# damaggu/StableKeypoints

Measured on AMD Instinct MI355X. Metric: images/sec (token-opt step, 512², N=500 tokens), higher is better.
Workload: dtype f32

## Files before the change

### include/skp.h

```cpp
#ifndef SKP_H
#define SKP_H

#ifdef __cplusplus
extern "C" {
#endif

#define SKP_OK 0
#define SKP_EBADARG (-1)
#define SKP_ELAUNCH (-2)
#define SKP_MAX_LAYERS 16

const char* skp_last_error(void);
int skp_version(void);

int skp_capture_fwd(const float* z_low, int BH, int s, int N, int R, float* attn, float* stats, void* stream);

int skp_capture_bwd(const float* z_low, int BH, int s, int N, int R, const float* dattn, int group, long long sb,
                    long long sp, long long sn, float gscale, const float* stats, float* dz_low, float* workspace,
                    void* stream);

int skp_capture_maps_fwd(const float* const* z_low, const int* sizes, int L, int B, int H, int N, int R, float* maps,
                         float* const* stats, void* stream);

int skp_capture_maps_bwd(const float* const* z_low, const int* sizes, int L, int B, int H, int N, int R,
                         const float* dmaps, float gscale, const float* const* stats, float* const* dz_low,
                         float* workspace, void* stream);

long long skp_capture_maps_bwd_sel_workspace(const int* sizes, int L, int B, int H, int N, int R, int K);
int skp_capture_maps_bwd_sel(const float* const* z_low, const int* sizes, int L, int B, int H, int N, int R,
                             const long long* sel_tok, int K, const float* gsel, float gscale,
                             const float* const* stats, float* const* dz_low, float* workspace, void* stream);
int skp_sel_bwd_timing(int enable);
int skp_sel_bwd_timing_read(double* ms, int* calls);

int skp_aggregate(const float* const* layers, int L, int BH, int RR, int N, const long long* indices,
                  int n_out, float* out, void* stream);

int skp_resize_bilinear(const float* in, int C, int R, int Ro, float* out, void* stream);
int skp_resize_bilinear_bwd(const float* gout, int C, int R, int Ro, float* gin, void* stream);

int skp_argmax2d(const float* maps, int T, int h, int w, const long long* rows, int n_rows, float* pos,
                 long long* idx, void* stream);

int skp_k_max_pixels(const float* maps, int T, int h, int w, int num, float radius2, float* pos,
                     float* masked, void* stream);

int skp_mask_radius(const float* maps, int T, int h, int w, const float* pos, float radius2, float* out,
                    void* stream);

int skp_weighted_avg(float* maps, int T, int h, int w, float distance, int mutate, float* pos, void* stream);

int skp_gaussian_target(const float* pos, int num, int T, int size, float sigma, float* out, void* stream);

int skp_topk_gaussian(const float* maps, int T, int h, int w, int top_k, float sigma, float epsilon,
                      int num_subjects, long long* out, double* kl, void* workspace, void* stream);

int skp_topk_gaussian_batch(const float* maps, int nb, int T, int h, int w, int top_k, float sigma,
                            float epsilon, int num_subjects, long long* out, double* kl, void* workspace,
                            void* stream);

int skp_topk_keys(const double* keys, int nb, int T, int top_k, long long* out, void* stream);

int skp_entropy_sort(const float* maps, int T, int h, int w, int top_k, long long* out, double* ent,
                     void* workspace, void* stream);

int skp_fps(const float* maps, int T, int h, int w, const long long* cand, int n_cand, int top_k,
            long long* out, int* n_out, void* workspace, void* stream);
int skp_fps_batch(const float* maps, int nb, int T, int h, int w, const long long* cand, int n_cand, int top_k,
                  long long* out, int* n_out, void* workspace, void* stream);
int skp_fps_keys_batch(const double* keys, const float* maps, int nb, int T, int h, int w, int n_cand, int top_k,
                       long long* cand, long long* out, int* n_out, void* workspace, void* stream);

int skp_sharpen_fwd(const float* A, int T, int h, int w, float sigma, int num_subjects, float* pos,
                     double* partial, float* loss, void* stream);
int skp_sharpen_bwd(const float* A, int T, int h, int w, float sigma, int num_subjects, const float* pos,
                     const float* gout, float* dA, void* stream);
int skp_sharpen_fwd_batch(const float* A, int nb, int T, int h, int w, float sigma, int num_subjects, float* pos,
                          double* partial, float* loss, void* stream);
int skp_sharpen_bwd_batch(const float* A, int nb, int T, int h, int w, float sigma, int num_subjects,
                          const float* pos, const float* gout, float* dA, void* stream);

int skp_affine_warp(const float* x, int B, int C, int H, int W, const float* theta, float* out, void* stream);
int skp_affine_warp_bwd(const float* gout, int B, int C, int H, int W, const float* theta, float* gin,
                        void* stream);

int skp_equiv_fwd(const float* A, const float* At, int T, int h, int w, const float* theta_inv,
                  double* partial, float* loss, void* stream);
int skp_equiv_bwd(const float* A, const float* At, int T, int h, int w, const float* theta_inv,
                  const float* gout, float* dA, float* dAt, void* stream);
int skp_equiv_fwd_batch(const float* A, const float* At, int nb, int T, int h, int w, const float* theta_inv,
                        double* partial, float* loss, void* stream);
int skp_equiv_bwd_batch(const float* A, const float* At, int nb, int T, int h, int w, const float* theta_inv,
                        const float* gout, float* dA, float* dAt, void* stream);

int skp_wino_in_transform(const float* x, int B, int C, int H, int W, float* V, void* stream);
int skp_wino_out_transform(const float* M, int B, int K, int H, int W, const float* bias, const float* residual,
                           float* y, void* stream);
int skp_wino_out_transform_kt(const float* M, int B, int K, int H, int W, const float* bias, const float* residual,
                              float* y, float* gn_part, void* stream);

int skp_bgemm_f32(const float* A, long long sAb, long long sAm, long long sAk, const float* B, long long sBb,
                  long long sBk, long long sBn, float* C, long long sCb, long long sCm, long long sCn, int batch,
                  int M, int N, int K, float alpha, int accumulate, void* stream);
int skp_bgemm_f32_2b(const float* A, long long sAo, long long sAb, long long sAm, long long sAk, const float* B,
                     long long sBo, long long sBb, long long sBk, long long sBn, float* C, long long sCo, long long sCb,
                     long long sCm, long long sCn, int batch, int hb, int M, int N, int K, float alpha, int accumulate,
                     void* stream);

int skp_groupnorm_workspace(int B, int C, long long HW, int G);
int skp_groupnorm_fwd(const float* x, const float* gamma, const float* beta, const float* shift, int B, int C,
                      long long HW, int G, float eps, int act, float* y, float* stats, double* partial,
                      void* stream);
int skp_groupnorm_bwd(const float* x, const float* dy, const float* gamma, const float* beta, const float* shift,
                      const float* stats, int B, int C, long long HW, int G, int act, float* dx, double* partial,
                      void* stream);
int skp_groupnorm_fwd_part(const float* x, const float* gamma, const float* beta, const float* shift, const float* part,
                           int nseg, int B, int C, long long HW, int G, float eps, int act, float* y, float* stats,
                           double* partial, void* stream);
int skp_groupnorm_stats(const float* x, const float* shift, int B, int C, long long HW, int G, float eps, float* stats,
                        double* partial, void* stream);
int skp_groupnorm_stats_part(const float* part, int nseg, const float* shift, int B, int C, long long HW, int G,
                             float eps, float* stats, double* partial, void* stream);
int skp_groupnorm_bwd_add(const float* x, const float* dy, const float* gamma, const float* beta, const float* shift,
                          const float* stats, int B, int C, long long HW, int G, int act, const float* dres, float* dx,
                          double* partial, void* stream);
int skp_softmax_bwd(const float* P, float* dP, long long rows, int cols, float alpha, void* stream);
int skp_softmax_fwd(float* S, long long rows, int cols, void* stream);
int skp_attn_dscore(const float* P, const float* dO, const float* V, const float* D, float* out, int BH, int S, int L,
                    int d, float alpha, void* stream);
int skp_attn_bwd_kv(const float* P, const float* dO, const float* Q, const float* V, const float* D, float* dS,
                    float* dV, float* dK, int BH, int S, int L, int d, float alpha, void* stream);
int skp_attn_fwd(const float* Q, const float* K, const float* V, float* O, float* stats, int BH, int S, int L, int d,
                 float scale, void* stream);
int skp_attn_bwd_flash(const float* Q, const float* K, const float* V, const float* dO, const float* stats,
                       const float* D, float* dS, float* dV, float* dK, int BH, int S, int L, int d, float scale,
                       void* stream);
int skp_attn_fwd_bshd(const float* Q, long long q_sb, int q_rs, const float* K, long long k_sb, int k_rs,
                      const float* V, long long v_sb, int v_rs, float* O, long long o_sb, int o_rs, float* stats, int B,
                      int H, int S, int L, int d, float scale, void* stream);
int skp_attn_bwd_flash_bshd(const float* Q, long long q_sb, int q_rs, const float* K, long long k_sb, int k_rs,
                            const float* V, long long v_sb, int v_rs, const float* dO, long long o_sb, int o_rs,
                            const float* stats, const float* D, float* dS, float* dV, long long dv_sb, int dv_rs,
                            float* dK, long long dk_sb, int dk_rs, int B, int H, int S, int L, int d, float scale,
                            void* stream);
int skp_layernorm_fwd(const float* x, const float* gamma, const float* beta, long long rows, int C, float eps, float* y,
                      float* stats, void* stream);
int skp_layernorm_bwd(const float* x, const float* dy, const float* gamma, const float* stats, long long rows, int C,
                      float* dx, void* stream);
int skp_layernorm_bwd_add(const float* x, const float* dy, const float* gamma, const float* stats, long long rows,
                          int C, const float* dres, float* dx, void* stream);
int skp_geglu_fwd(const float* h, long long rows, int I, float* out, void* stream);
int skp_geglu_bwd(const float* h, const float* dout, long long rows, int I, float* dh, void* stream);
int skp_residual_bias_add(const float* a, const float* h, const float* bias, int B, int C, long long HW,
                          float* out, void* stream);
int skp_wino_weights(const float* w, int K, int C, int flip, float* U, void* stream);
int skp_conv3x3_wino(const float* x, const float* U, const float* bias, const float* residual, float* y, int B, int C,
                     int K, int H, int W, int nsplit, float* ws, void* stream);
int skp_wino2_weights(const float* w, int K, int C, int flip, float* U, void* stream);
int skp_conv3x3_wino2(const float* x, const float* U, const float* bias, const float* residual, float* y, int B,
                      int C, int K, int H, int W, int nsplit, float* ws, void* stream);
int skp_conv3x3_wino2_gn(const float* x, const float* U, const float* bias, const float* residual, float* y, int B,
                         int C, int K, int H, int W, int nsplit, float* ws, float* gn_part, void* stream);
int skp_wino2_vtransform(const float* x, float* V, int B, int C, int H, int W, void* stream);
int skp_wino2_vtransform_gn(const float* x, const float* stats, const float* gamma, const float* beta,
                            const float* shift, int G, int act, float* V, int B, int C, int H, int W, void* stream);
int skp_conv3x3_wino2_v(const float* V, const float* U, const float* bias, const float* residual, float* y, int B,
                        int C, int K, int H, int W, int nsplit, float* ws, void* stream);
int skp_conv3x3_wino2_v_gn(const float* V, const float* U, const float* bias, const float* residual, float* y, int B,
                           int C, int K, int H, int W, int nsplit, float* ws, float* gn_part, void* stream);
int skp_wino2s2_weights(const float* w, int K, int C, float* U, void* stream);
int skp_conv3x3s2_f2(const float* x, const float* U, const float* bias, float* y, int B, int C, int K, int H, int W,
                     int nsplit, float* ws, void* stream);

int skp_map_range(const float* maps, int n, int h, int w, float* range, void* stream);
int skp_render_sheet(const float* images, int n, int H, int W, const float* maps, int h, int w, const float* range,
                     const float* lut, float alpha, const float* points, int K, float radius,
                     const unsigned char* colors, int rows, int cols, int f, int pad, unsigned char* out,
                     void* stream);

int skp_tta_reduce_workspace(int B, int n, int S);
int skp_tta_reduce(const float* maps, int B, int C, int n, int S, const float* theta_inv, float* pos, float* avg,
                   void* workspace, void* stream);

int skp_tta_reduce_scored_workspace(int B, int n, int S);
int skp_tta_reduce_scored(const float* maps, int B, int C, int n, int S, const float* theta_inv, float distance,
                          float* pos, float* refined, float* scores, float* avg, void* workspace, void* stream);

int skp_tta_reduce_peaks_workspace(int B, int n, int S, int num, float radius2);
int skp_tta_reduce_peaks(const float* maps, int B, int C, int n, int S, const float* theta_inv, int num,
                         float radius2, float* pos, float* values, float* avg, void* workspace, void* stream);
// ... 6 lines not shown
```

### stablekeypoints_amd/_lib.py

```python
import ctypes
import os

import torch

_HERE = os.path.dirname(os.path.abspath(__file__))
LIB_PATH = os.environ.get("SKP_LIB", os.path.join(_HERE, "libskp.so"))

_c_int, _c_float, _c_ll, _p = ctypes.c_int, ctypes.c_float, ctypes.c_longlong, ctypes.c_void_p

_SIGS = {
    "skp_capture_fwd": [_p, _c_int, _c_int, _c_int, _c_int, _p, _p, _p],
    "skp_capture_bwd": [_p, _c_int, _c_int, _c_int, _c_int, _p, _c_int, _c_ll, _c_ll, _c_ll, _c_float, _p, _p, _p,
                        _p],
    "skp_capture_maps_fwd": [ctypes.POINTER(_p), ctypes.POINTER(_c_int), _c_int, _c_int, _c_int, _c_int, _c_int, _p,
                             ctypes.POINTER(_p), _p],
    "skp_capture_maps_bwd": [ctypes.POINTER(_p), ctypes.POINTER(_c_int), _c_int, _c_int, _c_int, _c_int, _c_int, _p,
                             _c_float, ctypes.POINTER(_p), ctypes.POINTER(_p), _p, _p],
    "skp_capture_maps_bwd_sel": [ctypes.POINTER(_p), ctypes.POINTER(_c_int), _c_int, _c_int, _c_int, _c_int, _c_int,
                                 _p, _c_int, _p, _c_float, ctypes.POINTER(_p), ctypes.POINTER(_p), _p, _p],
    "skp_sel_bwd_timing": [_c_int],
    "skp_sel_bwd_timing_read": [_p, _p],
    "skp_capture_maps_bwd_sel_workspace": [ctypes.POINTER(_c_int), _c_int, _c_int, _c_int, _c_int, _c_int, _c_int],
    "skp_aggregate": [ctypes.POINTER(_p), _c_int, _c_int, _c_int, _c_int, _p, _c_int, _p, _p],
    "skp_resize_bilinear": [_p, _c_int, _c_int, _c_int, _p, _p],
    "skp_resize_bilinear_bwd": [_p, _c_int, _c_int, _c_int, _p, _p],
    "skp_argmax2d": [_p, _c_int, _c_int, _c_int, _p, _c_int, _p, _p, _p],
    "skp_k_max_pixels": [_p, _c_int, _c_int, _c_int, _c_int, _c_float, _p, _p, _p],
    "skp_mask_radius": [_p, _c_int, _c_int, _c_int, _p, _c_float, _p, _p],
    "skp_weighted_avg": [_p, _c_int, _c_int, _c_int, _c_float, _c_int, _p, _p],
    "skp_gaussian_target": [_p, _c_int, _c_int, _c_int, _c_float, _p, _p],
    "skp_topk_gaussian": [_p, _c_int, _c_int, _c_int, _c_int, _c_float, _c_float, _c_int, _p, _p, _p, _p],
    "skp_topk_gaussian_batch": [_p, _c_int, _c_int, _c_int, _c_int, _c_int, _c_float, _c_float, _c_int, _p, _p, _p,
                                _p],
    "skp_topk_keys": [_p, _c_int, _c_int, _c_int, _p, _p],
    "skp_entropy_sort": [_p, _c_int, _c_int, _c_int, _c_int, _p, _p, _p, _p],
    "skp_fps": [_p, _c_int, _c_int, _c_int, _p, _c_int, _c_int, _p, _p, _p, _p],
    "skp_fps_batch": [_p, _c_int, _c_int, _c_int, _c_int, _p, _c_int, _c_int, _p, _p, _p, _p],
    "skp_fps_keys_batch": [_p, _p, _c_int, _c_int, _c_int, _c_int, _c_int, _c_int, _p, _p, _p, _p, _p],
    "skp_sharpen_fwd": [_p, _c_int, _c_int, _c_int, _c_float, _c_int, _p, _p, _p, _p],
    "skp_sharpen_bwd": [_p, _c_int, _c_int, _c_int, _c_float, _c_int, _p, _p, _p, _p],
    "skp_wino_in_transform": [_p, _c_int, _c_int, _c_int, _c_int, _p, _p],
    "skp_wino_out_transform": [_p, _c_int, _c_int, _c_int, _c_int, _p, _p, _p, _p],
    "skp_wino_out_transform_kt": [_p, _c_int, _c_int, _c_int, _c_int, _p, _p, _p, _p, _p],
    "skp_sharpen_fwd_batch": [_p, _c_int, _c_int, _c_int, _c_int, _c_float, _c_int, _p, _p, _p, _p],
    "skp_sharpen_bwd_batch": [_p, _c_int, _c_int, _c_int, _c_int, _c_float, _c_int, _p, _p, _p, _p],
    "skp_affine_warp": [_p, _c_int, _c_int, _c_int, _c_int, _p, _p, _p],
    "skp_affine_warp_bwd": [_p, _c_int, _c_int, _c_int, _c_int, _p, _p, _p],
    "skp_equiv_fwd": [_p, _p, _c_int, _c_int, _c_int, _p, _p, _p, _p],
    "skp_equiv_bwd": [_p, _p, _c_int, _c_int, _c_int, _p, _p, _p, _p, _p],
    "skp_equiv_fwd_batch": [_p, _p, _c_int, _c_int, _c_int, _c_int, _p, _p, _p, _p],
    "skp_equiv_bwd_batch": [_p, _p, _c_int, _c_int, _c_int, _c_int, _p, _p, _p, _p, _p],
    "skp_bgemm_f32": [_p, _c_ll, _c_ll, _c_ll, _p, _c_ll, _c_ll, _c_ll, _p, _c_ll, _c_ll, _c_ll, _c_int, _c_int,
                      _c_int, _c_int, _c_float, _c_int, _p],
    "skp_bgemm_f32_2b": [_p, _c_ll, _c_ll, _c_ll, _c_ll, _p, _c_ll, _c_ll, _c_ll, _c_ll, _p, _c_ll, _c_ll, _c_ll,
                         _c_ll, _c_int, _c_int, _c_int, _c_int, _c_int, _c_float, _c_int, _p],
    "skp_groupnorm_workspace": [_c_int, _c_int, _c_ll, _c_int],
    "skp_groupnorm_fwd": [_p, _p, _p, _p, _c_int, _c_int, _c_ll, _c_int, _c_float, _c_int, _p, _p, _p, _p],
    "skp_groupnorm_bwd": [_p, _p, _p, _p, _p, _p, _c_int, _c_int, _c_ll, _c_int, _c_int, _p, _p, _p],
    "skp_groupnorm_bwd_add": [_p, _p, _p, _p, _p, _p, _c_int, _c_int, _c_ll, _c_int, _c_int, _p, _p, _p, _p],
    "skp_residual_bias_add": [_p, _p, _p, _c_int, _c_int, _c_ll, _p, _p],
    "skp_softmax_bwd": [_p, _p, _c_ll, _c_int, _c_float, _p],
    "skp_softmax_fwd": [_p, _c_ll, _c_int, _p],
    "skp_attn_dscore": [_p, _p, _p, _p, _p, _c_int, _c_int, _c_int, _c_int, _c_float, _p],
    "skp_attn_bwd_kv": [_p, _p, _p, _p, _p, _p, _p, _p, _c_int, _c_int, _c_int, _c_int, _c_float, _p],
    "skp_attn_fwd": [_p, _p, _p, _p, _p, _c_int, _c_int, _c_int, _c_int, _c_float, _p],
    "skp_attn_bwd_flash": [_p, _p, _p, _p, _p, _p, _p, _p, _p, _c_int, _c_int, _c_int, _c_int, _c_float, _p],
    "skp_attn_fwd_bshd": [_p, _c_ll, _c_int, _p, _c_ll, _c_int, _p, _c_ll, _c_int, _p, _c_ll, _c_int, _p, _c_int, _c_int,
                          _c_int, _c_int, _c_int, _c_float, _p],
    "skp_attn_bwd_flash_bshd": [_p, _c_ll, _c_int, _p, _c_ll, _c_int, _p, _c_ll, _c_int, _p, _c_ll, _c_int, _p, _p, _p,
                                _p, _c_ll, _c_int, _p, _c_ll, _c_int, _c_int, _c_int, _c_int, _c_int, _c_int, _c_float,
                                _p],
    "skp_layernorm_fwd": [_p, _p, _p, _c_ll, _c_int, _c_float, _p, _p, _p],
    "skp_layernorm_bwd": [_p, _p, _p, _p, _c_ll, _c_int, _p, _p],
    "skp_layernorm_bwd_add": [_p, _p, _p, _p, _c_ll, _c_int, _p, _p, _p],
    "skp_geglu_fwd": [_p, _c_ll, _c_int, _p, _p],
    "skp_geglu_bwd": [_p, _p, _c_ll, _c_int, _p, _p],
    "skp_wino_weights": [_p, _c_int, _c_int, _c_int, _p, _p],
    "skp_conv3x3_wino": [_p, _p, _p, _p, _p, _c_int, _c_int, _c_int, _c_int, _c_int, _c_int, _p, _p],
    "skp_wino2_weights": [_p, _c_int, _c_int, _c_int, _p, _p],
    "skp_conv3x3_wino2": [_p, _p, _p, _p, _p, _c_int, _c_int, _c_int, _c_int, _c_int, _c_int, _p, _p],
    "skp_conv3x3_wino2_gn": [_p, _p, _p, _p, _p, _c_int, _c_int, _c_int, _c_int, _c_int, _c_int, _p, _p, _p],
    "skp_groupnorm_fwd_part": [_p, _p, _p, _p, _p, _c_int, _c_int, _c_int, _c_ll, _c_int, _c_float, _c_int, _p, _p, _p,
                               _p],
    "skp_groupnorm_stats": [_p, _p, _c_int, _c_int, _c_ll, _c_int, _c_float, _p, _p, _p],
    "skp_groupnorm_stats_part": [_p, _c_int, _p, _c_int, _c_int, _c_ll, _c_int, _c_float, _p, _p, _p],
    "skp_wino2_vtransform": [_p, _p, _c_int, _c_int, _c_int, _c_int, _p],
    "skp_wino2_vtransform_gn": [_p, _p, _p, _p, _p, _c_int, _c_int, _p, _c_int, _c_int, _c_int, _c_int, _p],
    "skp_conv3x3_wino2_v": [_p, _p, _p, _p, _p, _c_int, _c_int, _c_int, _c_int, _c_int, _c_int, _p, _p],
    "skp_conv3x3_wino2_v_gn": [_p, _p, _p, _p, _p, _c_int, _c_int, _c_int, _c_int, _c_int, _c_int, _p, _p, _p],
    "skp_wino2s2_weights": [_p, _c_int, _c_int, _p, _p],
    "skp_conv3x3s2_f2":   [_p, _p, _p, _p, _c_int, _c_int, _c_int, _c_int, _c_int, _c_int, _p, _p],
    "skp_map_range": [_p, _c_int, _c_int, _c_int, _p, _p],
    "skp_render_sheet": [_p, _c_int, _c_int, _c_int, _p, _c_int, _c_int, _p, _p, _c_float, _p, _c_int, _c_float, _p,
                         _c_int, _c_int, _c_int, _c_int, _p, _p],
    "skp_tta_reduce_workspace": [_c_int, _c_int, _c_int],
    "skp_tta_reduce": [_p, _c_int, _c_int, _c_int, _c_int, _p, _p, _p, _p, _p],
    "skp_tta_reduce_scored_workspace": [_c_int, _c_int, _c_int],
    "skp_tta_reduce_scored": [_p, _c_int, _c_int, _c_int, _c_int, _p, _c_float, _p, _p, _p, _p, _p, _p],
    "skp_tta_reduce_peaks_workspace": [_c_int, _c_int, _c_int, _c_int, _c_float],
    "skp_tta_reduce_peaks": [_p, _c_int, _c_int, _c_int, _c_int, _p, _c_int, _c_float, _p, _p, _p, _p, _p],
    "skp_version": [],
}


_RESTYPE = {"skp_capture_maps_bwd_sel_workspace": _c_ll}
_MEASUREMENT_ONLY = {"skp_sel_bwd_timing", "skp_sel_bwd_timing_read"}


class SkpLibraryError(RuntimeError):
    pass


_lib = None


def lib():
    global _lib
    if _lib is None:
        if not os.path.exists(LIB_PATH):
            raise SkpLibraryError(f"libskp.so not found at {LIB_PATH}: build it with "
                                  "`python -c 'import __graft_entry__ as g; g.build()'` or `make -C stablekeypoints_amd/csrc`")
        try:
            L = ctypes.CDLL(LIB_PATH)
        except OSError as e:
            raise SkpLibraryError(f"cannot load {LIB_PATH}: {e}") from e
        for name, args in _SIGS.items():
            if name in _MEASUREMENT_ONLY and not hasattr(L, name):
                continue
            f = getattr(L, name)
            f.argtypes = args
            f.restype = _RESTYPE.get(name, _c_int)
        L.skp_last_error.argtypes = []
        L.skp_last_error.restype = ctypes.c_char_p
        _lib = L
    return _lib


def exported_symbols():
# ... 24 lines not shown
```

### stablekeypoints_amd/ops.py

```python
import ctypes
import os

import torch

from . import _lib
from ._lib import call, ptr, stream

F32 = torch.float32

_TIMER = None


def set_kernel_timer(timer):
    global _TIMER
    _TIMER = timer


class _NoTimer:
    def __enter__(self):
        return self

    def __exit__(self, *a):
        return False

# ... 1226 lines not shown

class QKVProjection(torch.autograd.Function):

    @staticmethod
    def forward(ctx, x, w3, C):
        out = torch.matmul(x, w3.t())
        ctx.save_for_backward(w3)
        ctx.C = C
        ctx.x_shape = x.shape
        ctx.set_materialize_grads(False)
        return tuple(out[..., i * C:(i + 1) * C] for i in range(w3.shape[0] // C))

    @staticmethod
    def backward(ctx, *grads):
        (w3,) = ctx.saved_tensors
        C = ctx.C
        dx = None
        for i, g in enumerate(grads):
            if g is None:
                continue
            g2 = g.reshape(-1, C)
            wi = w3[i * C:(i + 1) * C]
            if dx is None:
                dx = torch.mm(g2, wi)
            else:
                dx.addmm_(g2, wi)
        if dx is None:
            return None, None, None
        return dx.view(ctx.x_shape), None, None


QKV_FUSED = True


def qkv_projection(x, *ws):
    _lib.require_device(x)
    return QKVProjection.apply(x, _qkv_weight(*ws), int(ws[0].shape[0]))


class TokensProjIn(torch.autograd.Function):

    @staticmethod
    def forward(ctx, x, w, bias):
        B, C, HW = x.shape
        h = torch.bmm(x.transpose(1, 2), w.t().expand(B, C, w.shape[0]))
        if bias is not None:
            h.add_(bias)
        ctx.save_for_backward(w)
        return h

    @staticmethod
    def backward(ctx, dh):
        (w,) = ctx.saved_tensors
        B = dh.shape[0]
        dx = torch.bmm(w.t().expand(B, w.shape[1], w.shape[0]), dh.transpose(1, 2))
        return dx, None, None


class TokensProjOut(torch.autograd.Function):

    @staticmethod
    def forward(ctx, h, w):
        B = h.shape[0]
        ctx.save_for_backward(w)
        return torch.bmm(w.expand(B, *w.shape), h.transpose(1, 2))

    @staticmethod
    def backward(ctx, dy):
        (w,) = ctx.saved_tensors
        B = dy.shape[0]
        return torch.bmm(dy.transpose(1, 2), w.expand(B, *w.shape)), None


def tokens_proj_in(x, weight, bias):
    B, C = x.shape[:2]
    return TokensProjIn.apply(x.reshape(B, C, -1), weight.detach().reshape(weight.shape[0], C),
                              None if bias is None else bias.detach())


def tokens_proj_out(h, weight, bias, residual):
    B, C = residual.shape[:2]
    y = TokensProjOut.apply(h, weight.detach().reshape(C, h.shape[-1]))
    return residual_bias_add(residual, y.view(residual.shape), bias)


import weakref as _weakref

_WINO_U = {}
WINO_MIN_WORKGROUPS = 128
WINO_KERNEL = "auto"
WINO_SPLIT = True
WINO_NSPLIT_FORCE = 0


def _wino_v2(H, W, B=None):
    if WINO_KERNEL == "v1":
        return False
    return (H % 32 == 0 and W % 32 == 0) or (H == 16 and W == 16 and B is not None and B % 4 == 0)


def _wino_u_cached(weight, flip, form, build):
    key = id(weight)
    ent = _WINO_U.get(key)
    if ent is None or ent[0]() is not weight:
        ent = _WINO_U[key] = (_weakref.ref(weight, lambda _r: _WINO_U.pop(key, None)), {})
    hit = ent[1].get((flip, form))
    if hit is None or hit[0] != weight._version:
        hit = ent[1][(flip, form)] = (weight._version, build())
    return hit[1]


def _wino_u(weight, flip, v2=False):
    def build():
        w = _c(weight.detach())
        K, C = (w.shape[0], w.shape[1]) if not flip else (w.shape[1], w.shape[0])
        if v2 == "s2":
            U = torch.empty(K * C * 28, device=w.device, dtype=F32)
            call("skp_wino2s2_weights", ptr(w), K, C, ptr(U), stream(w.device))
        else:
            U = torch.empty(K * C * (40 if v2 else 36), device=w.device, dtype=F32)
            call("skp_wino2_weights" if v2 else "skp_wino_weights", ptr(w), K, C, int(flip), ptr(U), stream(w.device))
        return U
    return _wino_u_cached(weight, flip, v2, build)


def _batch_chunks(B, per_img_bytes):
    bmax = max(1, (2 ** 31 - 1) // per_img_bytes)
    for b0 in range(0, B, bmax):
        yield b0, min(B, b0 + bmax)


def _wino_plan_uncached(B, C, K, H, W, force):
    v2 = _wino_v2(H, W, B)
    if v2:
        wgs = (B // 4 if H == 16 else B * (H // 32) * (W // 32)) * (K // 32)
    elif B * (H // 4) * (W // 4) <= 32 and K % 64 == 0:
        wgs = K // 64
    else:
        wgs = -(-(B * (H // 4) * (W // 4)) // 64) * (K // 32)
    out_bytes = B * K * H * W * 4

    def cost(s):
        if v2:
            k = -(-2 * wgs * s // 256)
            st = C // s // 4
            return (k // 2) * st * 1.72e-6 + (k % 2) * st * 1.48e-6 + (s > 1) * (s + 1) * out_bytes / 2e12
        rounds = -(-wgs * s // 256)
        return rounds * ((C // s // 4) * 2.4e-6 + 5e-6) + (s > 1) * (s + 1) * out_bytes / 5e12

    nsplit = 1
    if WINO_SPLIT:
        cands = [s for s in range(1, 33) if C % (4 * s) == 0 and (s == 1 or C // s >= 32)]
        nsplit = min(cands, key=cost)
        if force and C % (4 * force) == 0:
            nsplit = force
    return v2, nsplit, wgs * nsplit


_WINO_PLANS = {}


def _wino_plan(B, C, K, H, W):
    force = int(WINO_NSPLIT_FORCE)
    key = (B, C, K, H, W, force, WINO_KERNEL, WINO_SPLIT)
    plan = _WINO_PLANS.get(key)
    if plan is None:
# ... 444 lines not shown
```

### stablekeypoints_amd/sd/unet.py

```python
import math

import os

import torch
import torch.nn as nn
import torch.nn.functional as F


class CaptureComplete(Exception):
    """Raised by a patched attention when its controller has every map it needs.

    The reference discards the UNet output of a capture pass
    (``ptp_utils.py:246-252``), and nothing after the 4th captured layer feeds the
    loss, so the forward may stop there (SURVEY.md §7 "UNet early exit").
    """


USE_FUSED_GROUPNORM = True
USE_SKP_LAYERNORM = True


def _fused(x, *modules):
    return USE_FUSED_GROUPNORM and x.is_cuda and not any(p.requires_grad for m in modules for p in m.parameters())

# ... 76 lines not shown
                qf = self.to_q(x)
                one = _shared_context(context)
                if one is not None:
                    k1, v1 = shared_kv(self, one)
                    kf, vf = k1.expand(x.shape[0], -1, -1), v1.expand(x.shape[0], -1, -1)
                else:
                    kf, vf = kv_projection(self, context)
            out = ops.attention_heads(qf, kf, vf, self.heads, self.scale)
            if out is None and one is not None and SHARED_HEAD_MAJOR and torch.is_grad_enabled():
                out = shared_context_attention(qf, k1, v1, self.heads, self.scale)
            if out is not None:
                return self.to_out[1](self.to_out[0](out))
            q = self.reshape_heads_to_batch_dim(qf)
            k, v = kf, vf
        else:
            q = self.reshape_heads_to_batch_dim(self.to_q(x))
            k, v = kv_projection(self, context)
        k = self.reshape_heads_to_batch_dim(k)
        v = self.reshape_heads_to_batch_dim(v)
        out = attention_core(q, k, v, self.scale, mask, self.heads)
        out = self.reshape_batch_dim_to_heads(out)
        return self.to_out[1](self.to_out[0](out))


SHARED_KV = True
SHARED_HEAD_MAJOR = True


def _shared_context(context):
    if SHARED_KV and context.dim() == 3 and context.shape[0] > 1 and context.stride(0) == 0:
        base = context._base
        if (base is not None and base.dim() == 3 and base.shape[0] == 1 and base.shape[1:] == context.shape[1:]
                and base.stride()[1:] == context.stride()[1:] and base.data_ptr() == context.data_ptr()):
            return base
        return context[:1]
    return None


def shared_kv(attn, one):
    from .. import ops
    if ops.QKV_FUSED and _fused(one, attn.to_k, attn.to_v) and attn.to_k.bias is None and attn.to_v.bias is None:
        return ops.qkv_projection(one, attn.to_k.weight, attn.to_v.weight)
    return attn.to_k(one), attn.to_v(one)


def shared_context_attention(qf, k1, v1, H, scale):
    B, S, C = qf.shape
    L, d = k1.shape[1], C // H
    q = qf.reshape(B, S, H, d).permute(2, 0, 1, 3).reshape(H, B * S, d)
    k = k1.reshape(L, H, d).transpose(0, 1).contiguous()
    v = v1.reshape(L, H, d).transpose(0, 1).contiguous()
    o = attention_core(q, k, v, scale)
    return o.reshape(H, B, S, d).permute(1, 2, 0, 3).reshape(B, S, C)


def kv_projection(attn, context):
    one = _shared_context(context)
    if one is not None:
        B = context.shape[0]
        k1, v1 = shared_kv(attn, one)
        return k1.expand(B, -1, -1), v1.expand(B, -1, -1)
    return attn.to_k(context), attn.to_v(context)


def attention_core(q, k, v, scale, mask=None, heads=1):
    if mask is None and CrossAttention.backend == "sdpa":
        return F.scaled_dot_product_attention(q.unsqueeze(0), k.unsqueeze(0), v.unsqueeze(0), scale=scale)[0]
    if mask is None and USE_FUSED_GROUPNORM and q.is_cuda and torch.is_grad_enabled() and \
            (q.requires_grad or k.requires_grad or v.requires_grad):
        from .. import ops
        return ops.math_attention(q, k, v, scale)
    if mask is None and USE_FUSED_GROUPNORM and q.is_cuda:
        from .. import ops
        return ops.attention_nograd(q, k, v, scale)
    sim = torch.baddbmm(torch.empty(q.shape[0], q.shape[1], k.shape[1], dtype=q.dtype, device=q.device),
                        q, k.transpose(1, 2), beta=0, alpha=scale)
    if mask is not None:
        b = mask.shape[0]
        m = mask.reshape(b, -1)[:, None, :].repeat(heads, 1, 1)
        sim = sim.masked_fill(~m, -torch.finfo(sim.dtype).max)
    return torch.bmm(sim.softmax(dim=-1), v)


class GEGLU(nn.Module):
    def __init__(self, dim_in, dim_out):
        super().__init__()
        self.proj = nn.Linear(dim_in, dim_out * 2)

    def forward(self, x):
        h = self.proj(x)
        if USE_FUSED_GROUPNORM and h.is_cuda:
            from .. import ops
            return ops.geglu(h)
        x, gate = h.chunk(2, dim=-1)
        return x * F.gelu(gate)


class FeedForward(nn.Module):
    def __init__(self, dim, mult=4, dropout=0.0):
        super().__init__()
        inner = dim * mult
        self.net = nn.ModuleList([GEGLU(dim, inner), nn.Dropout(dropout), nn.Linear(inner, dim)])

    def forward(self, x):
        for m in self.net:
            x = m(x)
        return x


class BasicTransformerBlock(nn.Module):
    def __init__(self, dim, n_heads, d_head, cross_attention_dim):
        super().__init__()
        self.attn1 = CrossAttention(dim, heads=n_heads, dim_head=d_head)
        self.ff = FeedForward(dim)
        self.attn2 = CrossAttention(dim, cross_attention_dim=cross_attention_dim, heads=n_heads, dim_head=d_head)
        self.norm1 = nn.LayerNorm(dim)
        self.norm2 = nn.LayerNorm(dim)
        self.norm3 = nn.LayerNorm(dim)

    def forward(self, h, context=None):
        y, h = _ln_res(self.norm1, h)
        h = self.attn1(y) + h
        y, h = _ln_res(self.norm2, h)
        h = self.attn2(y, context=context) + h
        y, h = _ln_res(self.norm3, h)
        return self.ff(y) + h


class Transformer2DModel(nn.Module):

    def __init__(self, num_attention_heads, attention_head_dim, in_channels, cross_attention_dim, norm_num_groups=32,
                 depth=1, linear_proj=False):
        super().__init__()
        inner = num_attention_heads * attention_head_dim
        self.linear_proj = linear_proj
        self.norm = nn.GroupNorm(norm_num_groups, in_channels, eps=1e-6, affine=True)
        self.proj_in = nn.Linear(in_channels, inner) if linear_proj else nn.Conv2d(in_channels, inner, 1)
        self.transformer_blocks = nn.ModuleList(
            [BasicTransformerBlock(inner, num_attention_heads, attention_head_dim, cross_attention_dim)
             for _ in range(depth)])
        self.proj_out = nn.Linear(inner, in_channels) if linear_proj else nn.Conv2d(inner, in_channels, 1)

    def forward(self, x, encoder_hidden_states=None):
        b, c, hh, ww = x.shape
        x, res = gn_act_res(self.norm, x, False)
        if not self.linear_proj and _fused(x, self.proj_in, self.proj_out):
            from .. import ops
            x = ops.tokens_proj_in(x, self.proj_in.weight, self.proj_in.bias)
            for blk in self.transformer_blocks:
                x = blk(x, context=encoder_hidden_states)
            return ops.tokens_proj_out(x, self.proj_out.weight, self.proj_out.bias, res)
        if self.linear_proj:
            x = self.proj_in(x.permute(0, 2, 3, 1).reshape(b, hh * ww, c))
        else:
            x = self.proj_in(x)
            x = x.permute(0, 2, 3, 1).reshape(b, hh * ww, x.shape[1])
        inner = x.shape[-1]
        for blk in self.transformer_blocks:
            x = blk(x, context=encoder_hidden_states)
        if self.linear_proj:
            return self.proj_out(x).reshape(b, hh, ww, c).permute(0, 3, 1, 2) + res
        x = x.reshape(b, hh, ww, inner).permute(0, 3, 1, 2)
        return self.proj_out(x) + res


class ResnetBlock2D(nn.Module):
    def __init__(self, in_channels, out_channels=None, temb_channels=1280, groups=32, eps=1e-5):
        super().__init__()
        out_channels = in_channels if out_channels is None else out_channels
        self.norm1 = nn.GroupNorm(groups, in_channels, eps=eps, affine=True)
        self.conv1 = nn.Conv2d(in_channels, out_channels, 3, 1, 1)
        self.time_emb_proj = nn.Linear(temb_channels, out_channels) if temb_channels is not None else None
        self.norm2 = nn.GroupNorm(groups, out_channels, eps=eps, affine=True)
        self.dropout = nn.Dropout(0.0)
        self.conv2 = nn.Conv2d(out_channels, out_channels, 3, 1, 1)
        self.conv_shortcut = nn.Conv2d(in_channels, out_channels, 1) if in_channels != out_channels else None

    def forward(self, x, temb=None):
        if _fused(x, self.conv1, self.conv2, self.norm2):
            from .. import ops
            vst = (not torch.is_grad_enabled() and x.dtype == torch.float32 and _fused(x, self.norm1)
                   and (self.dropout.p == 0 or not self.training))
            K = self.conv1.out_channels
            if vst and ops.gn_conv3x3_wins(x.shape[0], x.shape[1], K, x.shape[2], x.shape[3]):
                n1 = self.norm1
                h = ops.gn_conv3x3(x, n1.weight, n1.bias, n1.num_groups, n1.eps, True, None, self.conv1.weight)
            else:
                y, x = gn_act_res(self.norm1, x, True)
                h = ops.conv3x3(y, self.conv1.weight)
            shift = self.conv1.bias[None]
            if temb is not None and self.time_emb_proj is not None:
                shift = shift + self.time_emb_proj(F.silu(temb))
            bias = self.conv2.bias
            if self.conv_shortcut is not None:
                if _fused(x, self.conv_shortcut):
                    x = ops.conv1x1(x, self.conv_shortcut.weight)
                    bias = bias + self.conv_shortcut.bias
                else:
                    x = self.conv_shortcut(x)
            if vst and ops.gn_conv3x3_wins(h.shape[0], K, K, h.shape[2], h.shape[3]):
                n2 = self.norm2
                return ops.gn_conv3x3(h, n2.weight, n2.bias, n2.num_groups, n2.eps, True, shift, self.conv2.weight,
                                      bias, x)
            return ops.conv3x3(self.dropout(gn_act(self.norm2, h, True, shift)), self.conv2.weight, bias, x)
        h = self.conv1(gn_act(self.norm1, x, True))
        if temb is not None and self.time_emb_proj is not None:
            h = h + self.time_emb_proj(F.silu(temb))[:, :, None, None]
        h = self.conv2(self.dropout(gn_act(self.norm2, h, True)))
        if self.conv_shortcut is not None:
# ... 216 lines not shown
```

Measured before the change: 44.93.

## Add split-bf16 MFMA GEMM for frozen feed-forward linears with fused bias/residual

Adds a HIP GEMM that splits fp32 operands into three bf16 parts and runs six bf16 MFMA products per tile, emulating fp32 accuracy on matrix cores. Frozen weights are packed once and cached by identity and version, with a refresh kernel that rewrites only changed entries. The feed-forward GEGLU projection and output projection use it for a whitelisted set of shapes, with bias and residual fused into the epilogue, and the backward pass uses the transposed packed weight. The intent is to replace slower fp32 GEMMs with matrix-core work. In exchange it adds a repack launch per call and small numerical differences from true fp32.

```diff
diff --git a/include/skp.h b/include/skp.h
--- a/include/skp.h
+++ b/include/skp.h
@@ -106,6 +106,10 @@
                      long long sBo, long long sBb, long long sBk, long long sBn, float* C, long long sCo, long long sCb,
                      long long sCm, long long sCn, int batch, int hb, int M, int N, int K, float alpha, int accumulate,
                      void* stream);
+int skp_split_bf16_pack(const float* W, long long count, void* packed, int refresh, void* stream);
+int skp_gemm_split_f32(const float* A, long long lda, const void* packed, long long plane, long long ldw, int trans,
+                       const float* bias, const float* residual, long long ldr, float* C, long long ldc, int M, int N,
+                       int K, void* stream);
 
 int skp_groupnorm_workspace(int B, int C, long long HW, int G);
 int skp_groupnorm_fwd(const float* x, const float* gamma, const float* beta, const float* shift, int B, int C,
diff --git a/stablekeypoints_amd/_lib.py b/stablekeypoints_amd/_lib.py
--- a/stablekeypoints_amd/_lib.py
+++ b/stablekeypoints_amd/_lib.py
@@ -54,6 +54,8 @@
                       _c_int, _c_int, _c_float, _c_int, _p],
     "skp_bgemm_f32_2b": [_p, _c_ll, _c_ll, _c_ll, _c_ll, _p, _c_ll, _c_ll, _c_ll, _c_ll, _p, _c_ll, _c_ll, _c_ll,
                          _c_ll, _c_int, _c_int, _c_int, _c_int, _c_int, _c_float, _c_int, _p],
+    "skp_split_bf16_pack": [_p, _c_ll, _p, _c_int, _p],
+    "skp_gemm_split_f32": [_p, _c_ll, _p, _c_ll, _c_ll, _c_int, _p, _p, _c_ll, _p, _c_ll, _c_int, _c_int, _c_int, _p],
     "skp_groupnorm_workspace": [_c_int, _c_int, _c_ll, _c_int],
     "skp_groupnorm_fwd": [_p, _p, _p, _p, _c_int, _c_int, _c_ll, _c_int, _c_float, _c_int, _p, _p, _p, _p],
     "skp_groupnorm_bwd": [_p, _p, _p, _p, _p, _p, _c_int, _c_int, _c_ll, _c_int, _c_int, _p, _p, _p],
diff --git a/stablekeypoints_amd/csrc/skp_gemm_split.hip b/stablekeypoints_amd/csrc/skp_gemm_split.hip
--- /dev/null
+++ b/stablekeypoints_amd/csrc/skp_gemm_split.hip
@@ -0,0 +1,344 @@
+#include <algorithm>
+
+#include "skp_common.h"
+
+using namespace skp;
+
+namespace {
+
+typedef float f32x16 __attribute__((ext_vector_type(16)));
+typedef float f32x2 __attribute__((ext_vector_type(2)));
+typedef unsigned u32x4 __attribute__((ext_vector_type(4)));
+typedef __bf16 bf16x2 __attribute__((ext_vector_type(2)));
+typedef __bf16 bf16x8 __attribute__((ext_vector_type(8)));
+
+constexpr int BM = 128, BN = 128, BK = 32, NT = 256;
+constexpr int LDA = BK + 8;
+constexpr int PLANE = BM * LDA;
+constexpr int LDT = BN + 8;
+constexpr int TPLANE = (BK / 2) * LDT;
+constexpr int kBand = 8;
+constexpr int kOcc = 2;
+
+__device__ __forceinline__ unsigned pk_bf16(float lo, float hi) {
+  const f32x2 v = {lo, hi};
+  return __builtin_bit_cast(unsigned, __builtin_convertvector(v, bf16x2));
+}
+__device__ __forceinline__ float bf_lo(unsigned p) { return __uint_as_float(p << 16); }
+__device__ __forceinline__ float bf_hi(unsigned p) { return __uint_as_float(p & 0xffff0000u); }
+
+__device__ __forceinline__ void split2(float x, float y, unsigned& p0, unsigned& p1, unsigned& p2) {
+  p0 = pk_bf16(x, y);
+  x -= bf_lo(p0);
+  y -= bf_hi(p0);
+  p1 = pk_bf16(x, y);
+  x -= bf_lo(p1);
+  y -= bf_hi(p1);
+  p2 = pk_bf16(x, y);
+}
+
+template <bool REFRESH>
+__global__ __launch_bounds__(256) void split_pack_kernel(const float* __restrict__ W, unsigned short* __restrict__ P,
+                                                        long long quads, long long plane) {
+  const long long q = (long long)blockIdx.x * 256 + threadIdx.x;
+  if (q >= quads) return;
+  const float4 v = reinterpret_cast<const float4*>(W)[q];
+  uint2* d0 = reinterpret_cast<uint2*>(P + 4 * q);
+  uint2* d1 = reinterpret_cast<uint2*>(P + plane + 4 * q);
+  uint2* d2 = reinterpret_cast<uint2*>(P + 2 * plane + 4 * q);
+  uint2 o0, o1, o2;
+  if (REFRESH) {
+    o0 = *d0;
+    o1 = *d1;
+    o2 = *d2;
+  }
+  uint2 p0, p1, p2;
+  split2(v.x, v.y, p0.x, p1.x, p2.x);
+  split2(v.z, v.w, p0.y, p1.y, p2.y);
+  if (REFRESH && ((p0.x ^ o0.x) | (p0.y ^ o0.y) | (p1.x ^ o1.x) | (p1.y ^ o1.y) | (p2.x ^ o2.x) | (p2.y ^ o2.y)) == 0)
+    return;
+  *d0 = p0;
+  *d1 = p1;
+  *d2 = p2;
+}
+
+struct LoaderA {
+  float4 r[4];
+  unsigned off[4];
+  __device__ __forceinline__ void setup(int lda, int m0, int M) {
+#pragma unroll
+    for (int i = 0; i < 4; ++i) {
+      const int e = threadIdx.x + i * NT;
+      off[i] = min(m0 + (e >> 3), M - 1) * lda + 4 * (e & 7);
+    }
+  }
+  __device__ __forceinline__ void load(const float* __restrict__ A, int k0) {
+#pragma unroll
+    for (int i = 0; i < 4; ++i) r[i] = *reinterpret_cast<const float4*>(A + (off[i] + k0));
+  }
+  __device__ __forceinline__ void store(unsigned short* __restrict__ S) const {
+#pragma unroll
+    for (int i = 0; i < 4; ++i) {
+      const int e = threadIdx.x + i * NT;
+      uint2 p0, p1, p2;
+      split2(r[i].x, r[i].y, p0.x, p1.x, p2.x);
+      split2(r[i].z, r[i].w, p0.y, p1.y, p2.y);
+      unsigned short* d = S + (e >> 3) * LDA + 4 * (e & 7);
+      *reinterpret_cast<uint2*>(d) = p0;
+      *reinterpret_cast<uint2*>(d + PLANE) = p1;
+      *reinterpret_cast<uint2*>(d + 2 * PLANE) = p2;
+    }
+  }
+};
+
+template <bool TRANS>
+struct LoaderB {
+  u32x4 r[6];
+  unsigned off[2];
+  __device__ __forceinline__ void setup(int ldw, int n0, int N) {
+    const int s = threadIdx.x;
+    if (!TRANS) {
+      off[0] = min(n0 + (s >> 2), N - 1) * ldw + 8 * (s & 3);
+      off[1] = min(n0 + 64 + (s >> 2), N - 1) * ldw + 8 * (s & 3);
+    } else {
+      off[0] = 2 * (s >> 5) * ldw + min(n0 + 4 * (s & 31), N - 4);
+    }
+  }
+  __device__ __forceinline__ void load(const unsigned short* __restrict__ P, int plane, int ldw, int k0) {
+#pragma unroll
+    for (int i = 0; i < 6; ++i) {
+      if (!TRANS) {
+        r[i] = *reinterpret_cast<const u32x4*>(P + (off[i & 1] + ((i >> 1) * plane + k0)));
+      } else {
+        const unsigned short* q = P + (off[0] + ((i >> 1) * plane + (16 * (i & 1) + k0) * ldw));
+        const uint2 a = *reinterpret_cast<const uint2*>(q);
+        const uint2 b = *reinterpret_cast<const uint2*>(q + ldw);
+        r[i] = u32x4{a.x, a.y, b.x, b.y};
+      }
+    }
+  }
+  __device__ __forceinline__ void store(unsigned short* __restrict__ S) const {
+#pragma unroll
+    for (int i = 0; i < 6; ++i) {
+      const int e = threadIdx.x + i * NT;
+      const int p = e >> 9, s = e & 511;
+      if (!TRANS) {
+        *reinterpret_cast<u32x4*>(S + p * PLANE + (s >> 2) * LDA + 8 * (s & 3)) = r[i];
+      } else {
+        u32x4 v;
+        v.x = (r[i].x & 0xffffu) | (r[i].z << 16);
+        v.y = (r[i].x >> 16) | (r[i].z & 0xffff0000u);
+        v.z = (r[i].y & 0xffffu) | (r[i].w << 16);
+        v.w = (r[i].y >> 16) | (r[i].w & 0xffff0000u);
+        *reinterpret_cast<u32x4*>(reinterpret_cast<unsigned*>(S) + p * TPLANE + (s >> 5) * LDT + 4 * (s & 31)) = v;
+      }
+    }
+  }
+};
+
+__device__ __forceinline__ bf16x8 frag_rows(const unsigned short* __restrict__ S, int p, int t, int h, int mn) {
+  return __builtin_bit_cast(bf16x8, *reinterpret_cast<const uint4*>(S + p * PLANE + mn * LDA + 16 * t + 8 * h));
+}
+__device__ __forceinline__ bf16x8 frag_pairs(const unsigned short* __restrict__ S, int p, int t, int h, int n) {
+  const unsigned* q = reinterpret_cast<const unsigned*>(S) + p * TPLANE + (8 * t + 4 * h) * LDT + n;
+  return __builtin_bit_cast(bf16x8, make_uint4(q[0], q[LDT], q[2 * LDT], q[3 * LDT]));
+}
+
+template <bool TRANS, bool RES>
+__global__ __launch_bounds__(NT, kOcc) void gemm_split_kernel(const float* __restrict__ A, int lda,
+                                                              const unsigned short* __restrict__ P, int plane, int ldw,
+                                                              const float* __restrict__ bias,
+                                                              const float* __restrict__ R, int ldr,
+                                                              float* __restrict__ C, int ldc, int M, int N, int K,
+                                                              int tiles_n, int tiles) {
+  __shared__ __attribute__((aligned(16))) unsigned short As[3 * PLANE];
+  __shared__ __attribute__((aligned(16))) unsigned short Bs[3 * PLANE];
+  static_assert(3 * TPLANE * 4 <= 3 * PLANE * 2, "transposed image must fit the B buffer");
+  const int lane = threadIdx.x & 63, wid = threadIdx.x >> 6;
+  const int wm = (wid >> 1) * 64, wn = (wid & 1) * 64;
+  const int h = lane >> 5, r = lane & 31;
+  const int npanel = K / BK;
+  const int G = (int)gridDim.x >> 3;
+  const int per = (tiles + 7) / 8;
+  const int t0 = ((int)blockIdx.x & 7) * per + ((int)blockIdx.x >> 3);
+  const int span = min(tiles, ((int)blockIdx.x & 7) * per + per) - t0;
+  const int mine = span > 0 ? (span - 1) / G + 1 : 0;
+  if (mine == 0) return;
+  LoaderA la;
+  LoaderB<TRANS> lb;
+  struct Cursor {
+    int ti, p, m0, n0;
+  };
+  const int tiles_m = tiles / tiles_n;
+  auto tile_of = [&](int t, int& m0, int& n0) {
+    const int band = t / (kBand * tiles_n), rows = min(kBand, tiles_m - band * kBand);
+    const int u = t - band * kBand * tiles_n;
+    m0 = (band * kBand + u % rows) * BM;
+    n0 = (u / rows) * BN;
+  };
+  auto decode = [&](int ti, Cursor& c) {
+    c.ti = ti;
+    c.p = 0;
+    tile_of(t0 + ti * G, c.m0, c.n0);
+    if (!TRANS) la.setup(lda, c.m0, M);
+    lb.setup(ldw, c.n0, N);
+  };
+  Cursor ld;
+  decode(0, ld);
+  auto issue = [&]() {
+    if (TRANS) la.setup(lda, ld.m0, M);
+    la.load(A, ld.p * BK);
+    lb.load(P, plane, ldw, ld.p * BK);
+  };
+  auto advance = [&]() {
+    if (ld.p + 1 < npanel) ++ld.p;
+    else if (ld.ti + 1 < mine) decode(ld.ti + 1, ld);
+  };
+  issue();
+  advance();
+  la.store(As);
+  lb.store(Bs);
+  __syncthreads();
+  for (int ti = 0; ti < mine; ++ti) {
+    f32x16 acc[2][2], accs[2][2];
+#pragma unroll
+    for (int mi = 0; mi < 2; ++mi)
+#pragma unroll
+      for (int ni = 0; ni < 2; ++ni)
+#pragma unroll
+        for (int i = 0; i < 16; ++i) acc[mi][ni][i] = accs[mi][ni][i] = 0.0f;
+    for (int p = 0; p < npanel; ++p) {
+      issue();
+      advance();
+      __builtin_amdgcn_sched_barrier(0);
+#pragma unroll
+      for (int t = 0; t < BK / 16; ++t) {
+        bf16x8 a[2][3];
+#pragma unroll
+        for (int mi = 0; mi < 2; ++mi)
+#pragma unroll
+          for (int q = 0; q < 3; ++q) a[mi][q] = frag_rows(As, q, t, h, wm + 32 * mi + r);
+        constexpr int TA[6] = {0, 2, 1, 0, 1, 0};
+        constexpr int TB[6] = {2, 0, 1, 1, 0, 0};
+#pragma unroll
+        for (int ni = 0; ni < 2; ++ni) {
+          bf16x8 b[3];
+#pragma unroll
+          for (int q = 0; q < 3; ++q)
+            b[q] = TRANS ? frag_pairs(Bs, q, t, h, wn + 32 * ni + r) : frag_rows(Bs, q, t, h, wn + 32 * ni + r);
+#pragma unroll
+          for (int u = 0; u < 6; ++u)
+#pragma unroll
+            for (int mi = 0; mi < 2; ++mi) {
+              f32x16& c = u < 5 ? accs[mi][ni] : acc[mi][ni];
+              c = __builtin_amdgcn_mfma_f32_32x32x16_bf16(a[mi][TA[u]], b[TB[u]], c, 0, 0, 0);
+            }
+        }
+      }
+      __builtin_amdgcn_sched_barrier(0);
+      __syncthreads();
+      la.store(As);
+      lb.store(Bs);
+      if (p == npanel - 1) {
+        int tm0, tn0;
+        tile_of(t0 + ti * G, tm0, tn0);
+        int rb = tm0 + wm + 4 * h, cb = tn0 + wn + r;
+        asm volatile("" : "+v"(rb), "+v"(cb));
+        const bool full = tm0 + BM <= M && tn0 + BN <= N;
+#pragma unroll
+        for (int ni = 0; ni < 2; ++ni) {
+          const int col = cb + 32 * ni;
+          const float bv = bias ? bias[min(col, N - 1)] : 0.0f;
+#pragma unroll
+          for (int mi = 0; mi < 2; ++mi) {
+#pragma unroll
+            for (int hf = 0; hf < 2; ++hf) {
+              float rv[8];
+              if (RES) {
+#pragma unroll
+                for (int j = 0; j < 8; ++j) {
+                  const int row = rb + 32 * mi + (j & 3) + 8 * (2 * hf + (j >> 2));
+                  rv[j] = R[(unsigned)(min(row, M - 1) * ldr + min(col, N - 1))];
+                }
+              }
+              float v[8];
+#pragma unroll
+              for (int j = 0; j < 8; ++j) {
+                v[j] = (acc[mi][ni][8 * hf + j] + accs[mi][ni][8 * hf + j]) + bv;
+                if (RES) v[j] += rv[j];
+              }
+              if (full) {
+#pragma unroll
+                for (int j = 0; j < 8; ++j)
+                  C[(unsigned)((rb + 32 * mi + (j & 3) + 8 * (2 * hf + (j >> 2))) * ldc + col)] = v[j];
+              } else {
+#pragma unroll
+                for (int j = 0; j < 8; ++j) {
+                  const int row = rb + 32 * mi + (j & 3) + 8 * (2 * hf + (j >> 2));
+                  if (row < M && col < N) C[(unsigned)(row * ldc + col)] = v[j];
+                }
+              }
+              __builtin_amdgcn_sched_barrier(0);
+            }
+          }
+        }
+      }
+      __syncthreads();
+    }
+  }
+}
+
+bool aligned16(const void* p) { return (reinterpret_cast<uintptr_t>(p) & 15) == 0; }
+
+}
+
+extern "C" int skp_split_bf16_pack(const float* W, long long count, void* packed, int refresh, void* stream) {
+  SKP_CHECK_ARG(W && packed, "null pointer");
+  SKP_CHECK_ARG(count > 0 && count % 8 == 0, "count must be a positive multiple of 8");
+  SKP_CHECK_ARG(aligned16(W) && aligned16(packed), "pointers must be 16-byte aligned");
+  const long long quads = count / 4;
+  SKP_CHECK_ARG((quads + 255) / 256 < (1LL << 31), "too many elements");
+  const dim3 grid((unsigned)((quads + 255) / 256));
+  unsigned short* P = static_cast<unsigned short*>(packed);
+  if (refresh) hipLaunchKernelGGL(split_pack_kernel<true>, grid, dim3(256), 0, as_stream(stream), W, P, quads, count);
+  else hipLaunchKernelGGL(split_pack_kernel<false>, grid, dim3(256), 0, as_stream(stream), W, P, quads, count);
+  SKP_LAUNCH_CHECK();
+  return SKP_OK;
+}
+
+extern "C" int skp_gemm_split_f32(const float* A, long long lda, const void* packed, long long plane, long long ldw,
+                                  int trans, const float* bias, const float* residual, long long ldr, float* C,
+                                  long long ldc, int M, int N, int K, void* stream) {
+  SKP_CHECK_ARG(A && packed && C, "null pointer");
+  SKP_CHECK_ARG(M > 0 && N > 0 && K > 0, "non-positive shape");
+  SKP_CHECK_ARG(K % 32 == 0, "K must be a multiple of 32");
+  SKP_CHECK_ARG(N % 4 == 0, "N must be a multiple of 4");
+  SKP_CHECK_ARG(aligned16(A) && aligned16(packed) && aligned16(C) && aligned16(bias) && aligned16(residual),
+                "pointers must be 16-byte aligned");
+  SKP_CHECK_ARG(lda >= K && lda % 4 == 0, "lda must be a multiple of 4, at least K");
+  SKP_CHECK_ARG(ldc >= N && (!residual || ldr >= N), "ldc / ldr must be at least N");
+  SKP_CHECK_ARG(ldw == (trans ? N : K), "ldw must be the packed weight's row length");
+  SKP_CHECK_ARG(plane % 8 == 0 && plane >= (long long)N * K, "plane stride must be a multiple of 8, at least N*K");
+  const int tiles_m = (M + BM - 1) / BM, tiles_n = (N + BN - 1) / BN;
+  const long long tiles = (long long)tiles_m * tiles_n;
+  SKP_CHECK_ARG(tiles < (1LL << 30), "too many tiles");
+  SKP_CHECK_ARG((long long)M * lda < (1LL << 29) && (long long)M * ldc < (1LL << 29) && 3 * plane < (1LL << 30) &&
+                    (!residual || (long long)M * ldr < (1LL << 29)),
+                "operand larger than 2 GiB");
+  const int grid = (int)std::min<long long>(8 * ((tiles + 7) / 8), 256LL * kOcc);
+  hipStream_t st = as_stream(stream);
+  const unsigned short* P = static_cast<const unsigned short*>(packed);
+#define SKP_GS(T, RS)                                                                                            \
+  hipLaunchKernelGGL((gemm_split_kernel<T, RS>), dim3(grid), dim3(NT), 0, st, A, (int)lda, P, (int)plane, (int)ldw, bias,  \
+                     residual, (int)ldr, C, (int)ldc, M, N, K, tiles_n, (int)tiles)
+  if (trans) {
+    if (residual) SKP_GS(true, true);
+    else SKP_GS(true, false);
+  } else {
+    if (residual) SKP_GS(false, true);
+    else SKP_GS(false, false);
+  }
+#undef SKP_GS
+  SKP_LAUNCH_CHECK();
+  return SKP_OK;
+}
diff --git a/stablekeypoints_amd/ops.py b/stablekeypoints_amd/ops.py
--- a/stablekeypoints_amd/ops.py
+++ b/stablekeypoints_amd/ops.py
@@ -1332,6 +1332,98 @@
     B, C = residual.shape[:2]
     y = TokensProjOut.apply(h, weight.detach().reshape(C, h.shape[-1]))
     return residual_bias_add(residual, y.view(residual.shape), bias)
+
+
+GEMM_SPLIT = True
+
+GEMM_SPLIT_SHAPES = {
+    ("fwd", 32768, 2560, 320), ("fwd", 32768, 320, 1280), ("bwd", 32768, 1280, 320),
+    ("fwd", 8192, 5120, 640), ("fwd", 8192, 640, 2560), ("bwd", 8192, 2560, 640),
+    ("fwd", 2048, 10240, 1280),
+}
+
+_SPLIT_W = {}
+
+
+def gemm_split_ok(M, N, K):
+    return M > 0 and N > 0 and K > 0 and K % 32 == 0 and N % 4 == 0
+
+
+def _split_weight(w):
+    key = id(w)
+    sig = (w._version, w.data_ptr())
+    ent = _SPLIT_W.get(key)
+    wd = _c16(w.detach())
+    if ent is not None and ent[0] == sig and ent[1]() is w:
+        call("skp_split_bf16_pack", ptr(wd), wd.numel(), ptr(ent[2]), 1, stream(wd.device))
+        return ent[2]
+    packed = torch.empty((3,) + tuple(wd.shape), device=wd.device, dtype=torch.bfloat16)
+    call("skp_split_bf16_pack", ptr(wd), wd.numel(), ptr(packed), 0, stream(wd.device))
+    _SPLIT_W[key] = (sig, _weakref.ref(w, lambda _r, key=key: _SPLIT_W.pop(key, None)), packed)
+    return packed
+
+
+def split_weight_forget(w=None):
+    if w is None:
+        _SPLIT_W.clear()
+    else:
+        _SPLIT_W.pop(id(w), None)
+
+
+def gemm_split(a, packed, trans, bias=None, residual=None):
+    M, K = a.shape
+    N = packed.shape[2] if trans else packed.shape[1]
+    assert packed.shape[1 if trans else 2] == K, (a.shape, packed.shape, trans)
+    out = torch.empty(M, N, device=a.device, dtype=F32)
+    call("skp_gemm_split_f32", ptr(a), a.stride(0), ptr(packed), packed.stride(0), packed.stride(1), int(trans),
+         ptr(bias), ptr(residual), 0 if residual is None else residual.stride(0), ptr(out), N, M, N, K,
+         stream(a.device))
+    return out
+
+
+class LinearFrozen(torch.autograd.Function):
+
+    @staticmethod
+    def forward(ctx, x, w, packed, bias, residual, fwd, bwd):
+        N, K = w.shape
+        x2 = x.reshape(-1, K)
+        r2 = None if residual is None else residual.reshape(-1, N)
+        if fwd:
+            y = gemm_split(_c16(x2), packed, False, bias, None if r2 is None else _c16(r2))
+        else:
+            y = torch.nn.functional.linear(x2, w, bias)
+            y = y if r2 is None else y + r2
+        ctx.save_for_backward(packed if bwd else w)
+        ctx.bwd = bwd
+        ctx.x_shape = x.shape
+        ctx.has_res = residual is not None
+        return y.view(*x.shape[:-1], N)
+
+    @staticmethod
+    def backward(ctx, dy):
+        (w,) = ctx.saved_tensors
+        dx = None
+        if ctx.needs_input_grad[0]:
+            dy2 = dy.reshape(-1, dy.shape[-1])
+            dx = (gemm_split(_c16(dy2), w, True) if ctx.bwd else torch.mm(dy2, w)).view(ctx.x_shape)
+        return dx, None, None, None, (dy if ctx.has_res and ctx.needs_input_grad[4] else None), None, None
+
+
+def linear_frozen(x, weight, bias=None, residual=None, fwd=True, bwd=True):
+    _lib.require_device(x, weight)
+    N, K = weight.shape
+    if x.dtype != F32 or weight.dtype != F32 or not (gemm_split_ok(1, N, K) and gemm_split_ok(1, K, N)):
+        raise ValueError(f"linear_frozen needs fp32 and a weight (N, K) with both multiples of 32; got {x.dtype}, "
+                         f"{tuple(weight.shape)}")
+    packed = _split_weight(weight) if fwd or bwd else None
+    return LinearFrozen.apply(x, weight.detach(), packed, None if bias is None else _c16(bias.detach()), residual,
+                              bool(fwd), bool(bwd))
+
+
+def linear_frozen_wins(M, N, K):
+    if not GEMM_SPLIT:
+        return False, False
+    return ("fwd", M, N, K) in GEMM_SPLIT_SHAPES, ("bwd", M, K, N) in GEMM_SPLIT_SHAPES
 
 
 import weakref as _weakref
diff --git a/stablekeypoints_amd/sd/unet.py b/stablekeypoints_amd/sd/unet.py
--- a/stablekeypoints_amd/sd/unet.py
+++ b/stablekeypoints_amd/sd/unet.py
@@ -182,13 +182,24 @@
     return torch.bmm(sim.softmax(dim=-1), v)
 
 
+def _linear(linear, x, residual=None):
+    if x.dtype == torch.float32 and _fused(x, linear):
+        from .. import ops
+        N, K = linear.weight.shape
+        fwd, bwd = ops.linear_frozen_wins(x.numel() // K, N, K)
+        if fwd or bwd:
+            return ops.linear_frozen(x, linear.weight, linear.bias, residual, fwd, bwd)
+    y = linear(x)
+    return y if residual is None else y + residual
+
+
 class GEGLU(nn.Module):
     def __init__(self, dim_in, dim_out):
         super().__init__()
         self.proj = nn.Linear(dim_in, dim_out * 2)
 
     def forward(self, x):
-        h = self.proj(x)
+        h = _linear(self.proj, x)
         if USE_FUSED_GROUPNORM and h.is_cuda:
             from .. import ops
             return ops.geglu(h)
@@ -202,10 +213,10 @@
         inner = dim * mult
         self.net = nn.ModuleList([GEGLU(dim, inner), nn.Dropout(dropout), nn.Linear(inner, dim)])
 
-    def forward(self, x):
-        for m in self.net:
+    def forward(self, x, residual=None):
+        for m in self.net[:-1]:
             x = m(x)
-        return x
+        return _linear(self.net[-1], x, residual)
 
 
 class BasicTransformerBlock(nn.Module):
@@ -224,7 +235,7 @@
         y, h = _ln_res(self.norm2, h)
         h = self.attn2(y, context=context) + h
         y, h = _ln_res(self.norm3, h)
-        return self.ff(y) + h
+        return self.ff(y, residual=h)
 
 
 class Transformer2DModel(nn.Module):
```

Result: no change. 45.22, median of 6 (+0.6%).
